# Luoyadan/CRB-active-3Ddet

Hardware: AMD Instinct MI355X
Metric: frames/s SECOND fwd+bwd, KITTI 20k-pt clouds (higher is better)
Workload: dtype f32

## Files before the change

crb-active-3ddet_amd/csrc/rows_gemm4.hip:

```cpp
#include <atomic>
#include <type_traits>
#include <utility>
#include "crb_common.h"
#include "winograd_split.h"
#include "../../include/crb_hip.h"

typedef float f32x4 __attribute__((ext_vector_type(4)));

namespace {

constexpr int NT = 256;

template <typename F, int... I>
__device__ __forceinline__ void static_for_impl(F&& f, std::integer_sequence<int, I...>) {
  (f(std::integral_constant<int, I>{}), ...);
}
template <int N, typename F>
__device__ __forceinline__ void static_for(F&& f) { static_for_impl(f, std::make_integer_sequence<int, N>{}); }

template <int B>
__device__ __forceinline__ void mfma_acc(const bf16x8& A, const bf16x8& Bv) {
  asm volatile("v_mfma_f32_32x32x16_bf16 a[%2:%3], %0, %1, a[%2:%3]" : : "v"(A), "v"(Bv), "n"(B * 16), "n"(B * 16 + 15));
}
template <int R>
__device__ __forceinline__ float acc_read() {
  float x;
  asm volatile("v_accvgpr_read_b32 %0, a[%1]" : "=v"(x) : "n"(R));
  return x;
}
template <int R>
__device__ __forceinline__ void acc_zero() { asm volatile("v_accvgpr_write_b32 a[%0], 0" : : "n"(R)); }
__device__ __forceinline__ void acc_settle() { asm volatile("s_nop 15\n\ts_nop 15" ::: "memory"); }

#define RG_ACC_0_127                                                                                                                   \
  "a0", "a1", "a2", "a3", "a4", "a5", "a6", "a7", "a8", "a9", "a10", "a11", "a12", "a13", "a14", "a15", "a16", "a17", "a18", "a19",   \
      "a20", "a21", "a22", "a23", "a24", "a25", "a26", "a27", "a28", "a29", "a30", "a31", "a32", "a33", "a34", "a35", "a36", "a37",   \
      "a38", "a39", "a40", "a41", "a42", "a43", "a44", "a45", "a46", "a47", "a48", "a49", "a50", "a51", "a52", "a53", "a54", "a55",   \
      "a56", "a57", "a58", "a59", "a60", "a61", "a62", "a63", "a64", "a65", "a66", "a67", "a68", "a69", "a70", "a71", "a72", "a73",   \
      "a74", "a75", "a76", "a77", "a78", "a79", "a80", "a81", "a82", "a83", "a84", "a85", "a86", "a87", "a88", "a89", "a90", "a91",   \
      "a92", "a93", "a94", "a95", "a96", "a97", "a98", "a99", "a100", "a101", "a102", "a103", "a104", "a105", "a106", "a107", "a108", \
      "a109", "a110", "a111", "a112", "a113", "a114", "a115", "a116", "a117", "a118", "a119", "a120", "a121", "a122", "a123", "a124", \
      "a125", "a126", "a127"
#define RG_ACC_128_255                                                                                                                 \
  "a128", "a129", "a130", "a131", "a132", "a133", "a134", "a135", "a136", "a137", "a138", "a139", "a140", "a141", "a142", "a143",     \
      "a144", "a145", "a146", "a147", "a148", "a149", "a150", "a151", "a152", "a153", "a154", "a155", "a156", "a157", "a158", "a159", \
      "a160", "a161", "a162", "a163", "a164", "a165", "a166", "a167", "a168", "a169", "a170", "a171", "a172", "a173", "a174", "a175", \
      "a176", "a177", "a178", "a179", "a180", "a181", "a182", "a183", "a184", "a185", "a186", "a187", "a188", "a189", "a190", "a191", \
      "a192", "a193", "a194", "a195", "a196", "a197", "a198", "a199", "a200", "a201", "a202", "a203", "a204", "a205", "a206", "a207", \
      "a208", "a209", "a210", "a211", "a212", "a213", "a214", "a215", "a216", "a217", "a218", "a219", "a220", "a221", "a222", "a223", \
      "a224", "a225", "a226", "a227", "a228", "a229", "a230", "a231", "a232", "a233", "a234", "a235", "a236", "a237", "a238", "a239", \
      "a240", "a241", "a242", "a243", "a244", "a245", "a246", "a247", "a248", "a249", "a250", "a251", "a252", "a253", "a254", "a255"

__device__ constexpr int pass_a(int p) { return p == 0 ? 0 : p == 1 ? 2 : p == 2 ? 1 : p == 3 ? 0 : p == 4 ? 1 : 0; }
__device__ constexpr int pass_b(int p) { return p == 0 ? 2 : p == 1 ? 0 : p == 2 ? 1 : p == 3 ? 1 : 0; }

struct Split8 {
  float sv[2], s1[2], s2[2];
  u32x4 q0, q1, q2;
  template <int E>
  __device__ __forceinline__ void put(float v) {
    constexpr int hh = E & 1;
    sv[hh] = v;
    split3f(v, s1[hh], s2[hh]);
    if constexpr (hh == 1) {
      q0[E >> 1] = __builtin_amdgcn_perm(__float_as_uint(sv[1]), __float_as_uint(sv[0]), 0x07060302u);
      q1[E >> 1] = __builtin_amdgcn_perm(__float_as_uint(s1[1]), __float_as_uint(s1[0]), 0x07060302u);
      q2[E >> 1] = __builtin_amdgcn_perm(__float_as_uint(s2[1]), __float_as_uint(s2[0]), 0x07060302u);
    }
  }
  __device__ __forceinline__ void get(bf16x8 (&f)[3]) const {
    f[0] = __builtin_bit_cast(bf16x8, q0);
    f[1] = __builtin_bit_cast(bf16x8, q1);
    f[2] = __builtin_bit_cast(bf16x8, q2);
  }
};

__global__ __launch_bounds__(256) void rows_gemm4_weights_kernel(const float* __restrict__ w, int64_t s_ci, int64_t s_co, int64_t s_a,
                                                                 int64_t s_b, unsigned char* __restrict__ img, int cin, int cout, int s,
                                                                 int direction, int K, int N) {
  const int KS = K >> 4;
  const int64_t id = (int64_t)blockIdx.x * 256 + threadIdx.x;
  if (id >= (int64_t)(N >> 5) * KS * 64) return;
  const int lane = (int)(id & 63), r = lane & 31, h = lane >> 5;
  const int ks = (int)((id >> 6) % KS), nb = (int)((id >> 6) / KS);
  const int n = nb * 32 + r, k0 = (ks >> 1) * 32 + h * 16 + (ks & 1) * 8;
  u32x4 q[3];
  unsigned lo[3] = {0, 0, 0};
#pragma unroll
  for (int j = 0; j < 8; ++j) {
    const int k = k0 + j;
    const int ci = direction ? n : k, tc = direction ? k : n;
    const int t = tc / cout, co = tc - t * cout;
    const float v = w[ci * s_ci + co * s_co + (t / s) * s_a + (t % s) * s_b];
    unsigned p[3];
    split3(v, p[0], p[1], p[2]);
#pragma unroll
    for (int i = 0; i < 3; ++i) {
      if (j & 1) q[i][j >> 1] = lo[i] | (p[i] << 16);
      else lo[i] = p[i];
    }
  }
  unsigned char* dst = img + ((int64_t)(nb * KS + ks) * 3) * 1024 + lane * 16;
#pragma unroll
  for (int i = 0; i < 3; ++i) *reinterpret_cast<u32x4*>(dst + i * 1024) = q[i];
}

constexpr int RG_LDS_BYTES = 4 * 32 * 64 * 16;

struct RgArgs {
  const float* x;
  float* y;
  const unsigned char* wimg;
  int M;
  int W, s;
  int kseg, nseg;
  int tin, tout;
  int K, N;
  int ldx, ldy;
  int wrn;
  int col_tiles, tiles;
};

__device__ __forceinline__ unsigned big_pix(int m, int W, int s) { return (unsigned)(s * (m + (s - 1) * W * (m / W))); }

__global__ __launch_bounds__(NT, 1) void rows_gemm4_kernel(RgArgs a) {
  extern __shared__ __attribute__((aligned(16))) unsigned char rg_lds[];
  asm volatile("" ::: RG_ACC_0_127, RG_ACC_128_255);
  const int lane = threadIdx.x & 63, wave = __builtin_amdgcn_readfirstlane(threadIdx.x >> 6);
// ... 410 lines not shown
```

crb-active-3ddet_amd/pcdet/models/backbones_2d/base_bev_backbone.py:

```python
import numpy as np
import torch
import torch.nn as nn

from crbhip import bnrelu

from ...utils.fold_utils import fold_conv_bn
from ...utils.linear_rows import LinearRows, rows_view, rows_to_nchw


ROWS_TRAIN = True
ROWS_GEMM = True
WINOGRAD = __import__('os').environ.get('CRB_WINOGRAD', '1') != '0'


def _wino_fold(w, shift):
    from crbhip import winograd
    return winograd.weights_forward2(w), shift.contiguous()


def _wino_ok(conv, x, pad=None):
    if not WINOGRAD or not isinstance(conv, nn.Conv2d) or not x.is_cuda or x.dtype != torch.float32:
        return False
    from crbhip import winograd
    p = tuple(conv.padding) if pad is None else tuple(pad)
# ... 14 lines not shown
        layer_nums = list(model_cfg.get('LAYER_NUMS', None) or [])
        layer_strides = list(model_cfg.get('LAYER_STRIDES', None) or [])
        num_filters = list(model_cfg.get('NUM_FILTERS', None) or [])
        assert len(layer_nums) == len(layer_strides) == len(num_filters)
        upsample_strides = list(model_cfg.get('UPSAMPLE_STRIDES', None) or [])
        num_upsample_filters = list(model_cfg.get('NUM_UPSAMPLE_FILTERS', None) or [])
        assert len(upsample_strides) == len(num_upsample_filters)
        c_in_list = [input_channels] + num_filters[:-1]
        self.blocks = nn.ModuleList()
        self.deblocks = nn.ModuleList()
        for idx, (c_in, c_out, n, s) in enumerate(zip(c_in_list, num_filters, layer_nums, layer_strides)):
            layers = [nn.ZeroPad2d(1), nn.Conv2d(c_in, c_out, kernel_size=3, stride=s, padding=0, bias=False),
                      _bn(c_out), nn.ReLU()]
            for _ in range(n):
                layers += [nn.Conv2d(c_out, c_out, kernel_size=3, padding=1, bias=False), _bn(c_out), nn.ReLU()]
            self.blocks.append(nn.Sequential(*layers))
            if upsample_strides:
                us, uc = upsample_strides[idx], num_upsample_filters[idx]
                if us >= 1:
                    up = nn.ConvTranspose2d(c_out, uc, us, stride=us, bias=False)
                else:
                    ds = int(np.round(1 / us))
                    up = nn.Conv2d(c_out, uc, ds, stride=ds, bias=False)
                self.deblocks.append(nn.Sequential(up, _bn(uc), nn.ReLU()))
        c_in = sum(num_upsample_filters)
        if len(upsample_strides) > len(layer_nums):
            self.deblocks.append(nn.Sequential(
                nn.ConvTranspose2d(c_in, c_in, upsample_strides[-1], stride=upsample_strides[-1], bias=False),
                _bn(c_in), nn.ReLU()))
        self.num_bev_features = c_in

    @staticmethod
    def _run_folded(seq, x):
        mods = list(seq)
        i = 0
        while i < len(mods):
            m = mods[i]
            pad = None
            if isinstance(m, nn.ZeroPad2d) and i + 1 < len(mods) and isinstance(mods[i + 1], nn.Conv2d):
                c, pd = mods[i + 1], m.padding
                if c.padding == (0, 0) and c.padding_mode == 'zeros' and pd[0] == pd[1] and pd[2] == pd[3]:
                    pad, i, m = (pd[2], pd[0]), i + 1, c
            if isinstance(m, (nn.Conv2d, nn.ConvTranspose2d)) and i + 1 < len(mods) and isinstance(mods[i + 1], nn.BatchNorm2d):
                bn = mods[i + 1]
                relu = i + 2 < len(mods) and isinstance(mods[i + 2], nn.ReLU)
                if _wino_ok(m, x, pad):
                    from crbhip import winograd
                    U, shift = fold_conv_bn(m, bn, _wino_fold)
                    x = winograd.conv3x3_U2(x, U, shift, relu)
                    i += 3 if relu else 2
                    continue
                rows_ok = x.is_cuda and x.is_contiguous(memory_format=torch.channels_last) and m.bias is None
                if rows_ok:
                    y = m(x) if pad is None else torch.nn.functional.conv2d(x, m.weight, None, m.stride, pad, m.dilation,
                                                                             m.groups)
                    rows_ok = y.is_contiguous(memory_format=torch.channels_last) and \
                        bnrelu.supported(y.new_empty((2, y.shape[1])), bn)
                if rows_ok:
                    n, c, h, w_ = y.shape
                    rows = y.permute(0, 2, 3, 1).reshape(n * h * w_, c)
                    z = bnrelu.bn_apply_(rows, bn, relu)
                    x = z.view(n, h, w_, c).permute(0, 3, 1, 2)
                else:
                    w, shift = fold_conv_bn(m, bn)
                    if isinstance(m, nn.Conv2d):
                        x = torch.nn.functional.conv2d(x, w, shift, m.stride, m.padding if pad is None else pad, m.dilation,
                                                       m.groups)
                    else:
                        x = torch.nn.functional.conv_transpose2d(x, w, shift, m.stride, m.padding, m.output_padding,
                                                                 m.groups, m.dilation)
                    if relu:
                        x = torch.relu_(x)
                i += 3 if relu else 2
            else:
                x = m(x) if pad is None else torch.nn.functional.conv2d(x, m.weight, m.bias, m.stride, pad, m.dilation, m.groups)
                i += 1
        return x

    @staticmethod
    def _pad_conv(mods, i, x):
        m = mods[i]
        if isinstance(m, nn.ZeroPad2d) and i + 1 < len(mods) and isinstance(mods[i + 1], nn.Conv2d):
            c = mods[i + 1]
            pd = m.padding
            if c.padding == (0, 0) and c.padding_mode == 'zeros' and pd[0] == pd[1] and pd[2] == pd[3]:
                if _wino_ok(c, x, (pd[2], pd[0])):
                    from crbhip import winograd
                    return BaseBEVBackbone._wino_conv(c, x, mods[i + 2] if i + 2 < len(mods) else None), 2
                if torch.are_deterministic_algorithms_enabled() and torch.is_grad_enabled() and pd[0] == pd[2] and x.is_cuda:
                    from crbhip import dense_strided
                    if dense_strided.supported(c, x):
                        return dense_strided.conv_det(c, x, (pd[2], pd[0])), 2
                return torch.nn.functional.conv2d(x, c.weight, c.bias, c.stride, (pd[2], pd[0]), c.dilation, c.groups), 2
        return None, 0

    @staticmethod
    def _wino_conv(conv, x, nxt):
        from crbhip import winograd
        if winograd.STATS and conv.bias is None and isinstance(nxt, nn.BatchNorm2d) and nxt.training and \
                nxt.momentum is not None and bnrelu.FUSE_RUNNING and torch.is_grad_enabled() and not bnrelu.frame_groups_active():
            y, slabs = winograd.conv3x3_stats(x, conv.weight)
            y._crb_bn_slabs = slabs
            return y
        return winograd.conv3x3(x, conv.weight, conv.bias)

    @staticmethod
    def _run_rows_train(seq, x):
        mods = list(seq)
        i = 0
        while i < len(mods):
            m = mods[i]
            nxt = mods[i + 1] if i + 1 < len(mods) else None
            y, used = BaseBEVBackbone._pad_conv(mods, i, x)
            if used:
                x, i = y, i + used
                continue
            if _wino_ok(m, x):
                x = BaseBEVBackbone._wino_conv(m, x, nxt)
                i += 1
                continue
            if isinstance(m, nn.BatchNorm2d) and isinstance(nxt, nn.ReLU) and \
                    x.is_contiguous(memory_format=torch.channels_last) and \
                    bnrelu.supported(x.new_empty((2, x.shape[1])), m):
                n, c, h, w_ = x.shape
                rows = x.permute(0, 2, 3, 1).reshape(n * h * w_, c)
                slabs = getattr(x, '_crb_bn_slabs', None)
                x = bnrelu.bn_relu(rows, m, relu=True, slabs=slabs).view(n, h, w_, c).permute(0, 3, 1, 2)
                i += 2
            else:
                x = m(x)
                i += 1
        return x

    @staticmethod
    def _up(conv, x):
        if ROWS_GEMM and x.is_cuda:
            from crbhip import rows_gemm
            y = rows_gemm.up_conv(conv, x)
            if y is not None:
                return y
        if ROWS_GEMM and x.is_cuda and conv.bias is None and conv.kernel_size == (1, 1) and conv.stride == (1, 1) and \
# ... 98 lines not shown
```

include/crb_hip.h:

```cpp
#ifndef CRB_HIP_H
#define CRB_HIP_H
#include <stdint.h>

#ifdef __cplusplus
extern "C" {
#endif

#define CRB_OK 0
#define CRB_ERR_ARG (-1)
#define CRB_ERR_WORKSPACE (-2)
#define CRB_ERR_LAUNCH (-3)
#define CRB_ERR_UNSUPPORTED (-4)

int crb_abi_version(void);

int64_t crb_voxelize_workspace_bytes(int64_t n_points, int B, int max_voxels, int max_points);
int crb_voxelize(const float* points, int64_t n_points, int num_features,
                 const int32_t* frame_offsets, int B,
                 const float* range_min_xyz, const float* voxel_size_xyz, const int32_t* grid_xyz,
                 int max_voxels, int max_points,
                 float* voxels, int32_t* coords, int32_t* num_points, float* mean_features,
                 int32_t* num_voxels_out,
                 void* workspace, int64_t workspace_bytes, void* stream);

// ... 385 lines not shown
int64_t crb_winograd2_stats_slabs(int N, int H, int W);
int crb_conv3x3_winograd2_stats_nhwc(const float* x, const float* U, float* y, float* stats, int N, int H, int W, int cin, int cout,
                                     void* stream);

int crb_winograd4_supported(int cin, int cout, int H, int W);
int64_t crb_winograd4_weights_bytes(int cin, int cout);
int crb_winograd4_weights_conv(const float* w, int64_t so, int64_t si, int64_t sky, int64_t skx, void* U, int conv_cin, int conv_cout,
                               int mode, void* stream);
int crb_winograd4_weights_conv_multi(int n, const float* const* w, const int64_t* strides, void* const* U, const int32_t* conv_cin,
                                     const int32_t* conv_cout, const int32_t* mode, void* stream);
int crb_conv3x3_winograd4_nhwc(const float* x, const void* U, float* y, int N, int H, int W, int cin, int cout, const float* bias,
                               int relu, void* stream);
int64_t crb_winograd4_stats_slabs(int N, int H, int W);
int crb_conv3x3_winograd4_stats_nhwc(const float* x, const void* U, float* y, float* stats, int N, int H, int W, int cin, int cout,
                                     void* stream);
int crb_winograd4c_supported(int cin, int cout, int H, int W);
int crb_conv3x3_winograd4c_nhwc(const float* x, const void* U, float* y, int N, int H, int W, int cin, int cout,
                                const float* bias, int relu, void* stream);
int64_t crb_winograd4c_stats_slabs(int N, int H, int W);
int crb_conv3x3_winograd4c_stats_nhwc(const float* x, const void* U, float* y, float* stats, int N, int H, int W, int cin,
                                      int cout, void* stream);

int crb_bev_blocks_geometry(int N, int H, int W, int32_t* geom);
int64_t crb_bev_blocks_ints(int N, int H, int W);
int crb_bev_blocks(const int32_t* indices, int64_t n, int N, int H, int W, int32_t* out, int64_t out_ints, void* stream);
int crb_conv3x3_winograd4c_blocks_nhwc(const float* x, const void* U, float* y, float* stats, int N, int H, int W, int cin,
                                       int cout, const int32_t* list, const int32_t* count, const int32_t* rest,
                                       const int32_t* rest_count, void* stream);

int crb_winograd2_wgrad_supported(int cin, int cout, int H, int W);
int64_t crb_winograd2_wgrad_workspace_bytes(int cin, int cout);
int crb_winograd2_wgrad(const float* x, const float* dy, float* dw, int64_t so, int64_t si, int64_t sky, int64_t skx,
                        int N, int H, int W, int cin, int cout, void* workspace, int64_t workspace_bytes, void* stream);
int crb_winograd4_wgrad_supported(int cin, int cout, int H, int W);
int64_t crb_winograd4_wgrad_workspace_bytes(int cin, int cout);
int crb_winograd4_wgrad(const float* x, const float* dy, float* dw, int64_t so, int64_t si, int64_t sky, int64_t skx,
                        int N, int H, int W, int cin, int cout, void* workspace, int64_t workspace_bytes, void* stream);
int crb_winograd4_wgrad_blocks(const float* x, const float* dy, float* dw, int64_t so, int64_t si, int64_t sky, int64_t skx,
                               int N, int H, int W, int cin, int cout, const int32_t* list, const int32_t* count,
                               void* workspace, int64_t workspace_bytes, void* stream);

int crb_rows_gemm4_supported(int cin, int cout, int stride, int direction);
int64_t crb_rows_gemm4_weights_bytes(int cin, int cout, int stride);
int crb_rows_gemm4_weights(const float* w, int64_t s_ci, int64_t s_co, int64_t s_a, int64_t s_b, void* image, int cin, int cout,
                           int stride, int direction, void* stream);
int crb_rows_gemm4_forward(const float* x, const void* image, float* y, int N, int H, int W, int cin, int cout, int stride,
                           void* stream);
int crb_rows_gemm4_input_grad(const float* dy, const void* image, float* dx, int N, int H, int W, int cin, int cout, int stride,
                              void* stream);
int64_t crb_rows_gemm4_wgrad_workspace_bytes(int cin, int cout, int stride);
int crb_rows_gemm4_wgrad(const float* x, const float* dy, float* dw, int64_t s_ci, int64_t s_co, int64_t s_a, int64_t s_b, int N,
                         int H, int W, int cin, int cout, int stride, void* workspace, int64_t workspace_bytes, void* stream);

int crb_cu_reservation(int cus, void* stream);

int crb_bev_interpolate_forward(const float* bev, int B, int H, int W, int C, const float* keypoints, int64_t M, float x_min,
                                float y_min, float voxel_x, float voxel_y, float bev_stride, float* out, void* stream);
int crb_bev_interpolate_backward(const float* dout, int B, int H, int W, int C, const float* keypoints, int64_t M, float x_min,
                                 float y_min, float voxel_x, float voxel_y, float bev_stride, float* dbev, void* stream);

int crb_roi_bev_pool(const float* bev, int B, int H, int W, int C, const float* rois, int roi_row_stride, int R, int grid_size,
                     double x_min, double y_min, double cell_x, double cell_y, float* out, void* stream);

int crb_voxel_pool_supported(int C, int nsample);
int crb_voxel_query(const float* xyz, int64_t N, const float* new_xyz, const int32_t* new_coords, int64_t M, int B,
                    const int32_t* shape_dhw, const int32_t* ranges_zyx, float radius, int nsample, const int64_t* hkeys,
                    const int32_t* hvals, int64_t capacity, int32_t* idx, int32_t* cnt, void* stream);
int64_t crb_voxel_pool_moments_workspace_bytes(int64_t M);
int crb_voxel_pool_moments(const float* xyz, const float* new_xyz, const int32_t* idx, const int32_t* cnt, int64_t M, int nsample,
                           double* sums, void* workspace, int64_t workspace_bytes, void* stream);
int crb_voxel_pool_forward(const float* features_in, int64_t N, int C, const float* xyz, const float* new_xyz, const int32_t* idx,
                           const int32_t* cnt, int64_t M, int nsample, int pool, const float* A, const float* b, float* out,
                           void* stream);
int64_t crb_voxel_pool_backward_workspace_bytes(int64_t M, int C);
int crb_voxel_pool_backward(const float* grad_out, const float* features_in, int64_t N, int C, const float* xyz,
                            const float* new_xyz, const int32_t* idx, const int32_t* cnt, int64_t M, int nsample, int pool,
                            const float* A, const float* b, float* d_features, float* g_sel, int32_t* a_row, float* d_Ab,
                            void* workspace, int64_t workspace_bytes, void* stream);

int crb_pillar_vfe_supported(int C, int T, int Cout);
int crb_pillar_vfe_num_moments(int C);
int64_t crb_pillar_vfe_moments_workspace_bytes(int64_t M, int C);
int crb_pillar_vfe_moments(const float* voxels, const int32_t* num_points, const int32_t* coords, int64_t M, int T, int C,
                           const float* voxel_size, const float* offsets, double* sums, void* workspace, int64_t workspace_bytes,
                           void* stream);
int crb_pillar_vfe_forward(const float* voxels, const int32_t* num_points, const int32_t* coords, int64_t M, int T, int C,
                           const float* voxel_size, const float* offsets, const float* A, const float* b, int Cout, float* out,
                           void* stream);
int64_t crb_pillar_vfe_backward_workspace_bytes(int64_t M, int C, int Cout);
int crb_pillar_vfe_backward(const float* grad_out, const float* voxels, const int32_t* num_points, const int32_t* coords, int64_t M,
                            int T, int C, const float* voxel_size, const float* offsets, const float* A, const float* b, int Cout,
                            double* d_sums, void* workspace, int64_t workspace_bytes, void* stream);

#define CRB_LOSSNET_MAX_LAYERS 4
typedef struct CrbLossNetArgs {
  const float* x[CRB_LOSSNET_MAX_LAYERS];
  const float* w[CRB_LOSSNET_MAX_LAYERS];
  const float* gamma[CRB_LOSSNET_MAX_LAYERS];
  const float* beta[CRB_LOSSNET_MAX_LAYERS];
  float* running_mean[CRB_LOSSNET_MAX_LAYERS];
  float* running_var[CRB_LOSSNET_MAX_LAYERS];
  int64_t* num_batches_tracked[CRB_LOSSNET_MAX_LAYERS];
  int32_t channels[CRB_LOSSNET_MAX_LAYERS];
  int32_t num_layer;
  int32_t rows_per_frame;
  int32_t frames;
// ... 110 lines not shown
```

Baseline: 492.7.

## Add MFMA implicit-GEMM kernel for stride-2 3x3 convs in BEV backbone

Adds a custom HIP kernel for the bias-free 3x3 stride-2 padding-1 downsampling convolutions in the BEV backbone. It uses an implicit GEMM on bf16 MFMA with a three-way split of the f32 values, and handles the input gradient by decomposing it into four output-parity classes, each with its own tap subset. Weight images are cached per tensor version. By default only the input-gradient direction is switched on; forward and weight gradient still use the vendor convolution. Shared MFMA helpers move into a common header. The aim is to replace vendor strided-conv backward with a tuned kernel, at the cost of extra weight-image preparation and a more complex code path.

```diff
diff --git a/crb-active-3ddet_amd/crbhip/conv_s2.py b/crb-active-3ddet_amd/crbhip/conv_s2.py
--- /dev/null
+++ b/crb-active-3ddet_amd/crbhip/conv_s2.py
@@ -0,0 +1,204 @@
+import os
+
+import numpy as np
+import torch
+
+from ._lib import lib, check, ptr, cur_stream, require_cuda, CrbHipError
+
+KERNEL = os.environ.get('CRB_CONV_S2_KERNEL', 'x6')
+DEFAULT_LAUNCHES = 'i'
+LAUNCHES = set(v.strip() for v in os.environ.get('CRB_CONV_S2_LAUNCHES', DEFAULT_LAUNCHES).split(',') if v.strip())
+FORWARD, INPUT_GRAD, WGRAD = 0, 1, 2
+_DIR = 'fiw'
+TAPS_FORWARD = tuple((ky, kx) for ky in range(3) for kx in range(3))
+CLASSES = ((1, 1), (1, 0), (0, 1), (0, 0))
+
+
+def class_taps(ph, pw):
+    return tuple((ky, kx) for ky in ((0, 2) if ph else (1,)) for kx in ((0, 2) if pw else (1,)))
+
+
+TAPS_INPUT_GRAD = tuple(t for ph, pw in CLASSES for t in class_taps(ph, pw))
+
+
+def supported(cin, cout, direction):
+    return bool(lib.crb_conv_s2_supported(int(cin), int(cout), int(direction)))
+
+
+def use(cin, cout, direction):
+    return KERNEL == 'x6' and _DIR[direction] in LAUNCHES and supported(cin, cout, direction)
+
+
+def _geometry(conv, pad=None):
+    import torch.nn as nn
+    if not isinstance(conv, nn.Conv2d) or conv.bias is not None or conv.groups != 1 or conv.dilation != (1, 1):
+        return None
+    p = tuple(conv.padding) if pad is None else tuple(pad)
+    if conv.kernel_size != (3, 3) or conv.stride != (2, 2) or p != (1, 1) or conv.padding_mode != 'zeros':
+        return None
+    if pad is not None and tuple(conv.padding) != (0, 0):
+        return None
+    return conv.in_channels, conv.out_channels
+
+
+def dispatch(conv, x, pad=None):
+    g = _geometry(conv, pad)
+    if KERNEL != 'x6':
+        return 'vendor', 'CRB_CONV_S2_KERNEL=%s' % KERNEL
+    if g is None:
+        return 'vendor', 'not a bias-free 3x3 stride 2 padding 1 convolution'
+    if not (x.is_cuda and x.dim() == 4 and x.dtype == torch.float32 and x.is_contiguous(memory_format=torch.channels_last)):
+        return 'vendor', 'input is not an f32 channels_last device map'
+    cin, cout = g
+    if x.shape[1] != cin or x.shape[0] * x.shape[2] * x.shape[3] * max(cin, cout) >= 2 ** 31:
+        return 'vendor', 'map of %s does not fit the kernels\' 32-bit element index' % (tuple(x.shape),)
+    on = [d for d in range(3) if use(cin, cout, d)]
+    if not on:
+        return 'vendor', 'no direction of %d -> %d is switched on with an instance' % (cin, cout)
+    return 'x6', ''.join(_DIR[d] for d in on)
+
+
+_IMAGES = {}
+
+
+def weights(weight, cin, cout, direction):
+    require_cuda(weight)
+    w = weight.detach()
+    key = (w.data_ptr(), w.device.index, int(direction))
+    tag = (w._version, tuple(w.shape), tuple(w.stride()), cin, cout)
+    hit = _IMAGES.get(key)
+    if hit is not None and hit[0] == tag:
+        return hit[1]
+    if w.dtype != torch.float32 or tuple(w.shape) != (cout, cin, 3, 3):
+        raise CrbHipError('crb_conv_s2_weights takes an f32 (Cout, Cin, 3, 3) weight')
+    img = torch.empty((int(lib.crb_conv_s2_weights_bytes(cin, cout)),), dtype=torch.uint8, device=w.device)
+    s_co, s_ci, s_ky, s_kx = w.stride()
+    check(lib.crb_conv_s2_weights(w.data_ptr(), s_co, s_ci, s_ky, s_kx, ptr(img), cin, cout, int(direction), cur_stream(w.device)),
+          'crb_conv_s2_weights')
+    if len(_IMAGES) > 64:
+        _IMAGES.clear()
+    _IMAGES[key] = (tag, img, w)
+    return img
+
+
+def weight_matrix_reference(w, direction):
+    w = np.asarray(w)
+    if direction == FORWARD:
+        return np.concatenate([w[:, :, ky, kx].T for ky, kx in TAPS_FORWARD], axis=0)
+    return np.concatenate([w[:, :, ky, kx] for ky, kx in TAPS_INPUT_GRAD], axis=0)
+
+
+def weight_image_reference(w, direction):
+    wm = np.ascontiguousarray(weight_matrix_reference(np.asarray(w, dtype=np.float32), direction))
+    K, N = wm.shape
+    ks, lane, j = np.meshgrid(np.arange(K // 16), np.arange(64), np.arange(8), indexing='ij')
+    k = 32 * (ks >> 1) + 16 * (lane >> 5) + 8 * (ks & 1) + j
+    r = lane & 31
+    out = np.empty((N // 32, K // 16, 3, 64, 8), dtype=np.uint16)
+    for nb in range(N // 32):
+        v = np.ascontiguousarray(wm[k, 32 * nb + r])
+        for p in range(3):
+            hi = v.view(np.uint32) & np.uint32(0xffff0000)
+            out[nb, :, p] = (hi >> np.uint32(16)).astype(np.uint16)
+            v = v - hi.view(np.float32)
+    return out
+
+
+def forward_rows(N, H, W):
+    Ho, Wo = (H + 1) // 2, (W + 1) // 2
+    n, ho, wo = np.meshgrid(np.arange(N), np.arange(Ho), np.arange(Wo), indexing='ij')
+    src, valid = [], []
+    for ky, kx in TAPS_FORWARD:
+        h, w = 2 * ho - 1 + ky, 2 * wo - 1 + kx
+        valid.append(((h >= 0) & (h < H) & (w >= 0) & (w < W)).reshape(-1))
+        src.append(((n * H + np.clip(h, 0, H - 1)) * W + np.clip(w, 0, W - 1)).reshape(-1))
+    return np.stack(src), np.stack(valid)
+
+
+def input_grad_rows(N, H, W, ph, pw):
+    Ho, Wo = (H + 1) // 2, (W + 1) // 2
+    Hr, Wr = (H + 1 - ph) // 2, (W + 1 - pw) // 2
+    n, hr, wr = np.meshgrid(np.arange(N), np.arange(Hr), np.arange(Wr), indexing='ij')
+    dst = ((n * H + 2 * hr + ph) * W + 2 * wr + pw).reshape(-1)
+    src, valid = [], []
+    for ky, kx in class_taps(ph, pw):
+        ho, wo = hr + (1 if ky == 0 else 0), wr + (1 if kx == 0 else 0)
+        valid.append(((ho < Ho) & (wo < Wo)).reshape(-1))
+        src.append(((n * Ho + np.minimum(ho, Ho - 1)) * Wo + np.minimum(wo, Wo - 1)).reshape(-1))
+    return dst, np.stack(src), np.stack(valid)
+
+
+def _nhwc(x):
+    if not x.is_contiguous(memory_format=torch.channels_last):
+        x = x.contiguous(memory_format=torch.channels_last)
+    return x.permute(0, 2, 3, 1)
+
+
+def forward_x6(x, weight, cin, cout):
+    require_cuda(x, weight)
+    xv = _nhwc(x)
+    N, H, W, _ = xv.shape
+    img = weights(weight, cin, cout, FORWARD)
+    y = torch.empty((N, cout, (H + 1) // 2, (W + 1) // 2), dtype=torch.float32, device=x.device, memory_format=torch.channels_last)
+    check(lib.crb_conv_s2_forward(xv.data_ptr(), ptr(img), y.data_ptr(), N, H, W, cin, cout, cur_stream(x.device)), 'crb_conv_s2_forward')
+    return y
+
+
+def input_grad_x6(dy, weight, cin, cout, H, W):
+    require_cuda(dy, weight)
+    gv = _nhwc(dy)
+    N = gv.shape[0]
+    if tuple(gv.shape) != (N, (H + 1) // 2, (W + 1) // 2, cout):
+        raise CrbHipError('conv_s2 input gradient: dy does not belong to a %d x %d map' % (H, W))
+    img = weights(weight, cin, cout, INPUT_GRAD)
+    dx = torch.empty((N, cin, H, W), dtype=torch.float32, device=dy.device, memory_format=torch.channels_last)
+    check(lib.crb_conv_s2_input_grad(gv.data_ptr(), ptr(img), dx.data_ptr(), N, H, W, cin, cout, cur_stream(dy.device)),
+          'crb_conv_s2_input_grad')
+    return dx
+
+
+class _ConvS2(torch.autograd.Function):
+
+    @staticmethod
+    def forward(ctx, x, weight, cin, cout, det_wgrad=False):
+        ctx.save_for_backward(x, weight)
+        ctx.geo = (cin, cout)
+        ctx.det_wgrad = det_wgrad
+        if use(cin, cout, FORWARD):
+            return forward_x6(x, weight, cin, cout)
+        return torch.nn.functional.conv2d(x, weight, None, 2, 1)
+
+    @staticmethod
+    def backward(ctx, dy):
+        x, weight = ctx.saved_tensors
+        cin, cout = ctx.geo
+        dy = dy.contiguous(memory_format=torch.channels_last)
+        dx = dw = None
+        if ctx.needs_input_grad[0]:
+            if use(cin, cout, INPUT_GRAD):
+                dx = input_grad_x6(dy, weight, cin, cout, x.shape[2], x.shape[3])
+            else:
+                dx = torch.ops.aten.convolution_backward(dy, x, weight, None, [2, 2], [1, 1], [1, 1], False, [0, 0], 1,
+                                                         [True, False, False])[0]
+        if ctx.needs_input_grad[1]:
+            if ctx.det_wgrad:
+                from . import dense_strided
+                dw = dense_strided.weight_grad('conv', x, dy, 3, 3, 2, 1)
+            else:
+                dw = torch.ops.aten.convolution_backward(dy, x, weight, None, [2, 2], [1, 1], [1, 1], False, [0, 0], 1,
+                                                         [False, True, False])[1]
+        return dx, dw, None, None, None
+
+
+def conv(conv_module, x, pad=None):
+    path, _ = dispatch(conv_module, x, pad)
+    if path != 'x6':
+        return None
+    cin, cout = _geometry(conv_module, pad)
+    det_wgrad = False
+    if torch.are_deterministic_algorithms_enabled() and torch.is_grad_enabled():
+        from . import dense_strided
+        if not (use(cin, cout, FORWARD) and use(cin, cout, INPUT_GRAD) and dense_strided.supported(conv_module, x)):
+            return None
+        det_wgrad = True
+    return _ConvS2.apply(x, conv_module.weight, cin, cout, det_wgrad)
diff --git a/crb-active-3ddet_amd/csrc/conv_s2_rows.hip b/crb-active-3ddet_amd/csrc/conv_s2_rows.hip
--- /dev/null
+++ b/crb-active-3ddet_amd/csrc/conv_s2_rows.hip
@@ -0,0 +1,353 @@
+#include <atomic>
+#include <climits>
+#include "rows_gemm_common.h"
+#include "../../include/crb_hip.h"
+
+namespace {
+
+constexpr int CS_FLUSH = 8;
+constexpr int CS_LDS_BYTES = 4 * 32 * 64 * 16;
+constexpr int CS_SEGS = 4;
+
+__host__ constexpr int cs_geo(int nth, int ntw, int dh0, int sh, int dw0, int sw, int ph, int pw) {
+  return ntw | nth << 2 | (dh0 + 1) << 4 | (sh + 1) << 6 | (dw0 + 1) << 8 | (sw + 1) << 10 | ph << 12 | pw << 13;
+}
+
+struct CsArgs {
+  const float* x;
+  float* y;
+  const unsigned char* wimg;
+  int Hs, Ws, Hd, Wd;
+  int as, bs;
+  int kch, nch;
+  int wrn, col_tiles, tiles;
+  int tile0[CS_SEGS];
+  int M[CS_SEGS];
+  int Hr[CS_SEGS], Wr[CS_SEGS];
+  int geo[CS_SEGS];
+  int tap0[CS_SEGS];
+};
+
+struct CsSeg {
+  int tile0, M, Hr, Wr, ntw, dh0, sh, dw0, sw, ph, pw, KC, ks0;
+};
+
+__device__ __forceinline__ CsSeg cs_seg(const CsArgs& a, int tile) {
+  const int si = (tile >= a.tile0[1]) + (tile >= a.tile0[2]) + (tile >= a.tile0[3]);
+  auto pick = [&](const int (&v)[CS_SEGS]) __attribute__((always_inline)) { return si == 0 ? v[0] : si == 1 ? v[1] : si == 2 ? v[2] : v[3]; };
+  CsSeg s;
+  const int g = pick(a.geo);
+  s.tile0 = pick(a.tile0); s.M = pick(a.M); s.Hr = pick(a.Hr); s.Wr = pick(a.Wr); s.ks0 = pick(a.tap0) * (a.kch >> 4);
+  s.ntw = g & 3;
+  s.dh0 = ((g >> 4) & 3) - 1; s.sh = ((g >> 6) & 3) - 1;
+  s.dw0 = ((g >> 8) & 3) - 1; s.sw = ((g >> 10) & 3) - 1;
+  s.ph = (g >> 12) & 1; s.pw = (g >> 13) & 1;
+  s.KC = ((g >> 2) & 3) * s.ntw * (a.kch >> 5);
+  return s;
+}
+
+__global__ __launch_bounds__(NT, 1) void conv_s2_rows_kernel(CsArgs a) {
+  extern __shared__ __attribute__((aligned(16))) unsigned char cs_lds[];
+  asm volatile("" ::: RG_ACC_0_127, RG_ACC_128_255);
+  const int lane = threadIdx.x & 63, wave = __builtin_amdgcn_readfirstlane(threadIdx.x >> 6);
+  const int wr = wave % a.wrn, wc = wave / a.wrn, r = lane & 31, h = lane >> 5;
+  const int tile_rows = a.wrn * 64, tile_cols = (4 / a.wrn) * 128;
+  const int kcs = a.kch >> 5, KS = 18 * kcs;
+  int lt = blockIdx.x, lc = 0;
+  if (lt >= a.tiles) return;
+  const unsigned char* const wl = a.wimg + lane * 16;
+  CsSeg cur = cs_seg(a, lt);
+
+  static_for<256>([](auto rc) { acc_zero<decltype(rc)::value>(); });
+
+  int rn[2], rh[2], rw[2];
+  auto set_rows = [&](int tile, const CsSeg& s) __attribute__((always_inline)) {
+#pragma unroll
+    for (int rb = 0; rb < 2; ++rb) {
+      const int m = min(((tile - s.tile0) / a.col_tiles) * tile_rows + wr * 64 + rb * 32 + r, s.M - 1);
+      const int n = m / (s.Hr * s.Wr), rem = m - n * (s.Hr * s.Wr), hr = rem / s.Wr;
+      rn[rb] = n * a.Hs;
+      rh[rb] = a.as * hr;
+      rw[rb] = a.as * (rem - hr * s.Wr);
+    }
+  };
+  auto load_a = [&](int c, const CsSeg& s, f32x4 (&dst)[2][4], bool (&ok)[2]) __attribute__((always_inline)) {
+    const int t = c / kcs, cs = c - t * kcs, th = t / s.ntw, tw = t - th * s.ntw;
+    const int dh = s.dh0 + s.sh * th, dw = s.dw0 + s.sw * tw;
+#pragma unroll
+    for (int rb = 0; rb < 2; ++rb) {
+      const int hs = rh[rb] + dh, ws = rw[rb] + dw;
+      ok[rb] = (unsigned)hs < (unsigned)a.Hs && (unsigned)ws < (unsigned)a.Ws;
+      const int hc = min(max(hs, 0), a.Hs - 1), wcl = min(max(ws, 0), a.Ws - 1);
+      const float* p = a.x + ((size_t)(rn[rb] + hc) * a.Ws + wcl) * a.kch + cs * 32 + h * 16;
+#pragma unroll
+      for (int q = 0; q < 4; ++q) dst[rb][q] = *reinterpret_cast<const f32x4*>(p + 4 * q);
+    }
+  };
+  auto load_b = [&](int tile, const CsSeg& s, int ks, bf16x8 (&dst)[4][3]) __attribute__((always_inline)) {
+    const int nb0 = (((tile - s.tile0) % a.col_tiles) * tile_cols + wc * 128) >> 5;
+#pragma unroll
+    for (int cb = 0; cb < 4; ++cb)
+#pragma unroll
+      for (int p = 0; p < 3; ++p)
+        dst[cb][p] = *reinterpret_cast<const bf16x8*>(wl + ((size_t)((nb0 + cb) * KS + s.ks0 + ks) * 3 + p) * 1024);
+  };
+  auto step = [&](const bf16x8 (&Bw)[4][3], const bf16x8 (&Xf)[2][3], auto&& gap) __attribute__((always_inline)) {
+    static_for<48>([&](auto kc) __attribute__((always_inline)) {
+      constexpr int k = decltype(kc)::value, cb = k / 12, rb = (k / 6) & 1, pass = k % 6;
+      mfma_acc<(pass == 5 ? 0 : 8) + 4 * rb + cb>(Bw[cb][pass_a(pass)], Xf[rb][pass_b(pass)]);
+      gap(kc);
+      __builtin_amdgcn_sched_barrier(0);
+    });
+  };
+
+  f32x4 Ahi[2][2];
+  bool okhi[2];
+  bf16x8 XF0[2][3], B0[4][3];
+  set_rows(lt, cur);
+  {
+    f32x4 A0[2][4];
+    load_a(0, cur, A0, okhi);
+    load_b(lt, cur, 0, B0);
+#pragma unroll
+    for (int rb = 0; rb < 2; ++rb) {
+      Split8 sp;
+      static_for<8>([&](auto ec) { constexpr int e = decltype(ec)::value; sp.put<e>(okhi[rb] ? A0[rb][e >> 2][e & 3] : 0.f); });
+      sp.get(XF0[rb]);
+      Ahi[rb][0] = A0[rb][2];
+      Ahi[rb][1] = A0[rb][3];
+    }
+  }
+  asm volatile("s_nop 4" ::: "memory");
+
+  for (;;) {
+    int nt = lt, nc = lc + 1;
+    if (nc == cur.KC) { nc = 0; nt = lt + (int)gridDim.x; }
+    const bool more = nt < a.tiles;
+    if (!more) { nt = lt; nc = lc; }
+    CsSeg nxt = cur;
+    if (nt != lt) nxt = cs_seg(a, nt);
+    bf16x8 B1[4][3];
+    load_b(lt, cur, 2 * lc + 1, B1);
+    if (nt != lt) set_rows(nt, nxt);
+    f32x4 An[2][4];
+    bool okn[2];
+    load_a(nc, nxt, An, okn);
+    __builtin_amdgcn_sched_barrier(0);
+
+    bf16x8 XF1[2][3];
+    Split8 sp;
+    step(B0, XF0, [&](auto kc) __attribute__((always_inline)) {
+      constexpr int k = decltype(kc)::value;
+      if constexpr (k < 16) {
+        constexpr int rb = k >> 3, e = k & 7;
+        sp.put<e>(okhi[rb] ? Ahi[rb][e >> 2][e & 3] : 0.f);
+        if constexpr (e == 7) sp.get(XF1[rb]);
+      }
+    });
+    load_b(nt, nxt, 2 * nc, B0);
+    __builtin_amdgcn_sched_barrier(0);
+    step(B1, XF1, [&](auto kc) __attribute__((always_inline)) {
+      constexpr int k = decltype(kc)::value;
+      if constexpr (k >= 24 && k < 40) {
+        constexpr int rb = (k - 24) >> 3, e = (k - 24) & 7;
+        sp.put<e>(okn[rb] ? An[rb][e >> 2][e & 3] : 0.f);
+        if constexpr (e == 7) sp.get(XF0[rb]);
+      }
+    });
+
+    if (lc != cur.KC - 1 && (lc + 1) % CS_FLUSH == 0) {
+      f32x4* const part = reinterpret_cast<f32x4*>(cs_lds) + wave * (32 * 64) + lane;
+      const bool first = lc + 1 == CS_FLUSH;
+      acc_settle();
+      static_for<32>([&](auto qc) __attribute__((always_inline)) {
+        constexpr int R0 = 4 * decltype(qc)::value;
+        f32x4 v = (f32x4){acc_read<R0>(), acc_read<R0 + 1>(), acc_read<R0 + 2>(), acc_read<R0 + 3>()};
+        if (!first) v += part[decltype(qc)::value * 64];
+        part[decltype(qc)::value * 64] = v;
+      });
+      static_for<128>([](auto rc) { acc_zero<decltype(rc)::value>(); });
+      asm volatile("s_nop 4" ::: "memory");
+    }
+    if (lc == cur.KC - 1) {
+      const int tl = lt - cur.tile0;
+      const int col0 = (tl % a.col_tiles) * tile_cols + wc * 128;
+      const bool parts = cur.KC > CS_FLUSH;
+      acc_settle();
+      static_for<2>([&](auto rbc) __attribute__((always_inline)) {
+        constexpr int rb = decltype(rbc)::value;
+        const int m = (tl / a.col_tiles) * tile_rows + wr * 64 + rb * 32 + r;
+        const bool ok = m < cur.M;
+        const int mm = min(m, cur.M - 1);
+        const int n = mm / (cur.Hr * cur.Wr), rem = mm - n * (cur.Hr * cur.Wr), hr = rem / cur.Wr, wq = rem - hr * cur.Wr;
+        const int pix = (n * a.Hd + a.bs * hr + cur.ph) * a.Wd + a.bs * wq + cur.pw;
+        float* const out = a.y + (size_t)pix * a.nch + col0 + 4 * h;
+        static_for<16>([&](auto qc) __attribute__((always_inline)) {
+          constexpr int cb = decltype(qc)::value >> 2, j = decltype(qc)::value & 3, R0 = (4 * rb + cb) * 16 + 4 * j;
+          f32x4 v = (f32x4){acc_read<R0>() + acc_read<128 + R0>(), acc_read<R0 + 1>() + acc_read<129 + R0>(),
+                            acc_read<R0 + 2>() + acc_read<130 + R0>(), acc_read<R0 + 3>() + acc_read<131 + R0>()};
+          if (parts) v += (reinterpret_cast<const f32x4*>(cs_lds) + wave * (32 * 64) + lane)[(R0 / 4) * 64];
+          if (ok) *reinterpret_cast<f32x4*>(out + cb * 32 + 8 * j) = v;
+        });
+      });
+      static_for<256>([](auto rc) { acc_zero<decltype(rc)::value>(); });
+      asm volatile("s_nop 4" ::: "memory");
+    }
+    if (!more) break;
+#pragma unroll
+    for (int rb = 0; rb < 2; ++rb) {
+      Ahi[rb][0] = An[rb][2];
+      Ahi[rb][1] = An[rb][3];
+      okhi[rb] = okn[rb];
+    }
+    lt = nt;
+    lc = nc;
+    cur = nxt;
+  }
+}
+
+constexpr unsigned long long CS_ORDER_FWD = 0x876543210ULL;
+constexpr unsigned long long CS_ORDER_IGRAD = 0x453718620ULL;
+
+__global__ __launch_bounds__(256) void conv_s2_weights_kernel(const float* __restrict__ w, int64_t s_k, int64_t s_n, int64_t s_ky,
+                                                              int64_t s_kx, unsigned char* __restrict__ img, int kch, int nch,
+                                                              unsigned long long order) {
+  const int KS = (9 * kch) >> 4;
+  const int64_t id = (int64_t)blockIdx.x * 256 + threadIdx.x;
+  if (id >= (int64_t)(nch >> 5) * KS * 64) return;
+  const int lane = (int)(id & 63), r = lane & 31, h = lane >> 5;
+  const int ks = (int)((id >> 6) % KS), nb = (int)((id >> 6) / KS);
+  const int n = nb * 32 + r, k0 = (ks >> 1) * 32 + h * 16 + (ks & 1) * 8;
+  u32x4 q[3];
+  unsigned lo[3] = {0, 0, 0};
+#pragma unroll
+  for (int j = 0; j < 8; ++j) {
+    const int k = k0 + j;
+    const int t = k / kch, kc = k - t * kch, tap = (int)((order >> (4 * t)) & 15), ky = tap / 3, kx = tap - 3 * ky;
+    const float v = w[kc * s_k + n * s_n + ky * s_ky + kx * s_kx];
+    unsigned p[3];
+    split3(v, p[0], p[1], p[2]);
+#pragma unroll
+    for (int i = 0; i < 3; ++i) {
+      if (j & 1) q[i][j >> 1] = lo[i] | (p[i] << 16);
+      else lo[i] = p[i];
+    }
+  }
+  unsigned char* dst = img + ((int64_t)(nb * KS + ks) * 3) * 1024 + lane * 16;
+#pragma unroll
+  for (int i = 0; i < 3; ++i) *reinterpret_cast<u32x4*>(dst + i * 1024) = q[i];
+}
+
+__host__ int cs_cu_count() {
+  static std::atomic<int> n_cu{0};
+  int n = n_cu.load(std::memory_order_relaxed);
+  if (!n) {
+    int dev = 0;
+    hipDeviceProp_t prop;
+    if (hipGetDevice(&dev) != hipSuccess || hipGetDeviceProperties(&prop, dev) != hipSuccess) return 256;
+    n = prop.multiProcessorCount > 0 ? prop.multiProcessorCount : 256;
+    n_cu.store(n, std::memory_order_relaxed);
+  }
+  return n;
+}
+
+__host__ bool cs_sizes_ok(int N, int H, int W, int cin, int cout) {
+  if (N <= 0 || H <= 0 || W <= 0) return false;
+  return (int64_t)N * H * W * (cin > cout ? cin : cout) < (1LL << 31);
+}
+
+constexpr int CS_PH[CS_SEGS] = {1, 1, 0, 0}, CS_PW[CS_SEGS] = {1, 0, 1, 0};
+
+__host__ int cs_launch(CsArgs& a, int nsegs, void* stream) {
+  a.wrn = a.nch % 256 == 0 ? 2 : 4;
+  const int tile_rows = a.wrn * 64, tile_cols = (4 / a.wrn) * 128;
+  a.col_tiles = a.nch / tile_cols;
+  int64_t tiles = 0;
+  for (int s = 0; s < CS_SEGS; ++s) {
+    if (s >= nsegs) { a.tile0[s] = INT_MAX; a.M[s] = 0; a.Hr[s] = a.Wr[s] = 1; a.geo[s] = a.geo[0]; a.tap0[s] = 0; continue; }
+    a.tile0[s] = (int)tiles;
+    tiles += (((int64_t)a.M[s] + tile_rows - 1) / tile_rows) * a.col_tiles;
+    if (tiles >= (1LL << 30)) return CRB_ERR_ARG;
+  }
+  a.tiles = (int)tiles;
+  if (!a.tiles) return CRB_OK;
+  const int grid = a.tiles < cs_cu_count() ? a.tiles : cs_cu_count();
+  static std::atomic<unsigned> attr_done[64];
+  int dev = 0;
+  CRB_HIP(hipGetDevice(&dev));
+  if (dev < 0 || dev >= 64) return CRB_ERR_ARG;
+  if (!attr_done[dev].load(std::memory_order_acquire)) {
+    CRB_HIP(hipFuncSetAttribute((const void*)conv_s2_rows_kernel, hipFuncAttributeMaxDynamicSharedMemorySize, CS_LDS_BYTES));
+    attr_done[dev].store(1u, std::memory_order_release);
+  }
+  hipLaunchKernelGGL(conv_s2_rows_kernel, dim3((unsigned)grid), dim3(NT), CS_LDS_BYTES, (hipStream_t)stream, a);
+  CRB_CHECK_LAUNCH();
+  return CRB_OK;
+}
+
+}
+
+extern "C" int crb_conv_s2_supported(int cin, int cout, int direction) {
+  const bool n_ok = cout == 128 || cout == 256;
+  if (direction == 0) return ((cin == 64 || cin == 128) && n_ok) ? 1 : 0;
+  if (direction == 1) return (cin == 128 && n_ok) ? 1 : 0;
+  return 0;
+}
+
+extern "C" int64_t crb_conv_s2_weights_bytes(int cin, int cout) {
+  if (!crb_conv_s2_supported(cin, cout, 0) && !crb_conv_s2_supported(cin, cout, 1)) return 0;
+  return (int64_t)9 * cin * cout * 6;
+}
+
+extern "C" int crb_conv_s2_weights(const float* w, int64_t s_co, int64_t s_ci, int64_t s_ky, int64_t s_kx, void* image, int cin, int cout,
+                                   int direction, void* stream) {
+  if (direction != 0 && direction != 1) return CRB_ERR_ARG;
+  if (!crb_conv_s2_supported(cin, cout, direction)) return CRB_ERR_UNSUPPORTED;
+  if (!w || !image) return CRB_ERR_ARG;
+  const int kch = direction ? cout : cin, nch = direction ? cin : cout;
+  const int64_t threads = (int64_t)(nch / 32) * (9 * kch / 16) * 64;
+  hipLaunchKernelGGL(conv_s2_weights_kernel, dim3((unsigned)((threads + 255) / 256)), dim3(256), 0, (hipStream_t)stream, w,
+                     direction ? s_co : s_ci, direction ? s_ci : s_co, s_ky, s_kx, (unsigned char*)image, kch, nch,
+                     direction ? CS_ORDER_IGRAD : CS_ORDER_FWD);
+  CRB_CHECK_LAUNCH();
+  return CRB_OK;
+}
+
+extern "C" int crb_conv_s2_forward(const float* x, const void* image, float* y, int N, int H, int W, int cin, int cout, void* stream) {
+  if (N <= 0 || H <= 0 || W <= 0 || !x || !image || !y) return CRB_ERR_ARG;
+  if (!crb_conv_s2_supported(cin, cout, 0)) return CRB_ERR_UNSUPPORTED;
+  if (!cs_sizes_ok(N, H, W, cin, cout)) return CRB_ERR_ARG;
+  const int Ho = (H + 1) / 2, Wo = (W + 1) / 2;
+  CsArgs a;
+  a.x = x; a.y = y; a.wimg = (const unsigned char*)image;
+  a.Hs = H; a.Ws = W; a.Hd = Ho; a.Wd = Wo;
+  a.as = 2; a.bs = 1;
+  a.kch = cin; a.nch = cout;
+  a.M[0] = N * Ho * Wo; a.Hr[0] = Ho; a.Wr[0] = Wo;
+  a.geo[0] = cs_geo(3, 3, -1, 1, -1, 1, 0, 0);
+  a.tap0[0] = 0;
+  return cs_launch(a, 1, stream);
+}
+
+extern "C" int crb_conv_s2_input_grad(const float* dy, const void* image, float* dx, int N, int H, int W, int cin, int cout,
+                                      void* stream) {
+  if (N <= 0 || H <= 0 || W <= 0 || !dy || !image || !dx) return CRB_ERR_ARG;
+  if (!crb_conv_s2_supported(cin, cout, 1)) return CRB_ERR_UNSUPPORTED;
+  if (!cs_sizes_ok(N, H, W, cin, cout)) return CRB_ERR_ARG;
+  const int Ho = (H + 1) / 2, Wo = (W + 1) / 2;
+  CsArgs a;
+  a.x = dy; a.y = dx; a.wimg = (const unsigned char*)image;
+  a.Hs = Ho; a.Ws = Wo; a.Hd = H; a.Wd = W;
+  a.as = 1; a.bs = 2;
+  a.kch = cout; a.nch = cin;
+  int tap0 = 0;
+  for (int s = 0; s < CS_SEGS; ++s) {
+    const int ph = CS_PH[s], pw = CS_PW[s];
+    const int Hr = (H + 1 - ph) / 2, Wr = (W + 1 - pw) / 2;
+    a.M[s] = N * Hr * Wr; a.Hr[s] = Hr > 0 ? Hr : 1; a.Wr[s] = Wr > 0 ? Wr : 1;
+    a.geo[s] = cs_geo(1 + ph, 1 + pw, ph, -1, pw, -1, ph, pw);
+    a.tap0[s] = tap0;
+    tap0 += (1 + ph) * (1 + pw);
+  }
+  return cs_launch(a, CS_SEGS, stream);
+}
diff --git a/crb-active-3ddet_amd/csrc/rows_gemm4.hip b/crb-active-3ddet_amd/csrc/rows_gemm4.hip
--- a/crb-active-3ddet_amd/csrc/rows_gemm4.hip
+++ b/crb-active-3ddet_amd/csrc/rows_gemm4.hip
@@ -5,75 +5,9 @@
 #include "winograd_split.h"
 #include "../../include/crb_hip.h"
 
-typedef float f32x4 __attribute__((ext_vector_type(4)));
+#include "rows_gemm_common.h"
 
 namespace {
-
-constexpr int NT = 256;
-
-template <typename F, int... I>
-__device__ __forceinline__ void static_for_impl(F&& f, std::integer_sequence<int, I...>) {
-  (f(std::integral_constant<int, I>{}), ...);
-}
-template <int N, typename F>
-__device__ __forceinline__ void static_for(F&& f) { static_for_impl(f, std::make_integer_sequence<int, N>{}); }
-
-template <int B>
-__device__ __forceinline__ void mfma_acc(const bf16x8& A, const bf16x8& Bv) {
-  asm volatile("v_mfma_f32_32x32x16_bf16 a[%2:%3], %0, %1, a[%2:%3]" : : "v"(A), "v"(Bv), "n"(B * 16), "n"(B * 16 + 15));
-}
-template <int R>
-__device__ __forceinline__ float acc_read() {
-  float x;
-  asm volatile("v_accvgpr_read_b32 %0, a[%1]" : "=v"(x) : "n"(R));
-  return x;
-}
-template <int R>
-__device__ __forceinline__ void acc_zero() { asm volatile("v_accvgpr_write_b32 a[%0], 0" : : "n"(R)); }
-__device__ __forceinline__ void acc_settle() { asm volatile("s_nop 15\n\ts_nop 15" ::: "memory"); }
-
-#define RG_ACC_0_127                                                                                                                   \
-  "a0", "a1", "a2", "a3", "a4", "a5", "a6", "a7", "a8", "a9", "a10", "a11", "a12", "a13", "a14", "a15", "a16", "a17", "a18", "a19",   \
-      "a20", "a21", "a22", "a23", "a24", "a25", "a26", "a27", "a28", "a29", "a30", "a31", "a32", "a33", "a34", "a35", "a36", "a37",   \
-      "a38", "a39", "a40", "a41", "a42", "a43", "a44", "a45", "a46", "a47", "a48", "a49", "a50", "a51", "a52", "a53", "a54", "a55",   \
-      "a56", "a57", "a58", "a59", "a60", "a61", "a62", "a63", "a64", "a65", "a66", "a67", "a68", "a69", "a70", "a71", "a72", "a73",   \
-      "a74", "a75", "a76", "a77", "a78", "a79", "a80", "a81", "a82", "a83", "a84", "a85", "a86", "a87", "a88", "a89", "a90", "a91",   \
-      "a92", "a93", "a94", "a95", "a96", "a97", "a98", "a99", "a100", "a101", "a102", "a103", "a104", "a105", "a106", "a107", "a108", \
-      "a109", "a110", "a111", "a112", "a113", "a114", "a115", "a116", "a117", "a118", "a119", "a120", "a121", "a122", "a123", "a124", \
-      "a125", "a126", "a127"
-#define RG_ACC_128_255                                                                                                                 \
-  "a128", "a129", "a130", "a131", "a132", "a133", "a134", "a135", "a136", "a137", "a138", "a139", "a140", "a141", "a142", "a143",     \
-      "a144", "a145", "a146", "a147", "a148", "a149", "a150", "a151", "a152", "a153", "a154", "a155", "a156", "a157", "a158", "a159", \
-      "a160", "a161", "a162", "a163", "a164", "a165", "a166", "a167", "a168", "a169", "a170", "a171", "a172", "a173", "a174", "a175", \
-      "a176", "a177", "a178", "a179", "a180", "a181", "a182", "a183", "a184", "a185", "a186", "a187", "a188", "a189", "a190", "a191", \
-      "a192", "a193", "a194", "a195", "a196", "a197", "a198", "a199", "a200", "a201", "a202", "a203", "a204", "a205", "a206", "a207", \
-      "a208", "a209", "a210", "a211", "a212", "a213", "a214", "a215", "a216", "a217", "a218", "a219", "a220", "a221", "a222", "a223", \
-      "a224", "a225", "a226", "a227", "a228", "a229", "a230", "a231", "a232", "a233", "a234", "a235", "a236", "a237", "a238", "a239", \
-      "a240", "a241", "a242", "a243", "a244", "a245", "a246", "a247", "a248", "a249", "a250", "a251", "a252", "a253", "a254", "a255"
-
-__device__ constexpr int pass_a(int p) { return p == 0 ? 0 : p == 1 ? 2 : p == 2 ? 1 : p == 3 ? 0 : p == 4 ? 1 : 0; }
-__device__ constexpr int pass_b(int p) { return p == 0 ? 2 : p == 1 ? 0 : p == 2 ? 1 : p == 3 ? 1 : 0; }
-
-struct Split8 {
-  float sv[2], s1[2], s2[2];
-  u32x4 q0, q1, q2;
-  template <int E>
-  __device__ __forceinline__ void put(float v) {
-    constexpr int hh = E & 1;
-    sv[hh] = v;
-    split3f(v, s1[hh], s2[hh]);
-    if constexpr (hh == 1) {
-      q0[E >> 1] = __builtin_amdgcn_perm(__float_as_uint(sv[1]), __float_as_uint(sv[0]), 0x07060302u);
-      q1[E >> 1] = __builtin_amdgcn_perm(__float_as_uint(s1[1]), __float_as_uint(s1[0]), 0x07060302u);
-      q2[E >> 1] = __builtin_amdgcn_perm(__float_as_uint(s2[1]), __float_as_uint(s2[0]), 0x07060302u);
-    }
-  }
-  __device__ __forceinline__ void get(bf16x8 (&f)[3]) const {
-    f[0] = __builtin_bit_cast(bf16x8, q0);
-    f[1] = __builtin_bit_cast(bf16x8, q1);
-    f[2] = __builtin_bit_cast(bf16x8, q2);
-  }
-};
 
 __global__ __launch_bounds__(256) void rows_gemm4_weights_kernel(const float* __restrict__ w, int64_t s_ci, int64_t s_co, int64_t s_a,
                                                                  int64_t s_b, unsigned char* __restrict__ img, int cin, int cout, int s,
diff --git a/crb-active-3ddet_amd/csrc/rows_gemm_common.h b/crb-active-3ddet_amd/csrc/rows_gemm_common.h
--- /dev/null
+++ b/crb-active-3ddet_amd/csrc/rows_gemm_common.h
@@ -0,0 +1,77 @@
+#pragma once
+#include <type_traits>
+#include <utility>
+#include "crb_common.h"
+#include "winograd_split.h"
+
+typedef float f32x4 __attribute__((ext_vector_type(4)));
+
+namespace {
+
+constexpr int NT = 256;
+
+template <typename F, int... I>
+__device__ __forceinline__ void static_for_impl(F&& f, std::integer_sequence<int, I...>) {
+  (f(std::integral_constant<int, I>{}), ...);
+}
+template <int N, typename F>
+__device__ __forceinline__ void static_for(F&& f) { static_for_impl(f, std::make_integer_sequence<int, N>{}); }
+
+template <int B>
+__device__ __forceinline__ void mfma_acc(const bf16x8& A, const bf16x8& Bv) {
+  asm volatile("v_mfma_f32_32x32x16_bf16 a[%2:%3], %0, %1, a[%2:%3]" : : "v"(A), "v"(Bv), "n"(B * 16), "n"(B * 16 + 15));
+}
+template <int R>
+__device__ __forceinline__ float acc_read() {
+  float x;
+  asm volatile("v_accvgpr_read_b32 %0, a[%1]" : "=v"(x) : "n"(R));
+  return x;
+}
+template <int R>
+__device__ __forceinline__ void acc_zero() { asm volatile("v_accvgpr_write_b32 a[%0], 0" : : "n"(R)); }
+__device__ __forceinline__ void acc_settle() { asm volatile("s_nop 15\n\ts_nop 15" ::: "memory"); }
+
+#define RG_ACC_0_127                                                                                                                   \
+  "a0", "a1", "a2", "a3", "a4", "a5", "a6", "a7", "a8", "a9", "a10", "a11", "a12", "a13", "a14", "a15", "a16", "a17", "a18", "a19",   \
+      "a20", "a21", "a22", "a23", "a24", "a25", "a26", "a27", "a28", "a29", "a30", "a31", "a32", "a33", "a34", "a35", "a36", "a37",   \
+      "a38", "a39", "a40", "a41", "a42", "a43", "a44", "a45", "a46", "a47", "a48", "a49", "a50", "a51", "a52", "a53", "a54", "a55",   \
+      "a56", "a57", "a58", "a59", "a60", "a61", "a62", "a63", "a64", "a65", "a66", "a67", "a68", "a69", "a70", "a71", "a72", "a73",   \
+      "a74", "a75", "a76", "a77", "a78", "a79", "a80", "a81", "a82", "a83", "a84", "a85", "a86", "a87", "a88", "a89", "a90", "a91",   \
+      "a92", "a93", "a94", "a95", "a96", "a97", "a98", "a99", "a100", "a101", "a102", "a103", "a104", "a105", "a106", "a107", "a108", \
+      "a109", "a110", "a111", "a112", "a113", "a114", "a115", "a116", "a117", "a118", "a119", "a120", "a121", "a122", "a123", "a124", \
+      "a125", "a126", "a127"
+#define RG_ACC_128_255                                                                                                                 \
+  "a128", "a129", "a130", "a131", "a132", "a133", "a134", "a135", "a136", "a137", "a138", "a139", "a140", "a141", "a142", "a143",     \
+      "a144", "a145", "a146", "a147", "a148", "a149", "a150", "a151", "a152", "a153", "a154", "a155", "a156", "a157", "a158", "a159", \
+      "a160", "a161", "a162", "a163", "a164", "a165", "a166", "a167", "a168", "a169", "a170", "a171", "a172", "a173", "a174", "a175", \
+      "a176", "a177", "a178", "a179", "a180", "a181", "a182", "a183", "a184", "a185", "a186", "a187", "a188", "a189", "a190", "a191", \
+      "a192", "a193", "a194", "a195", "a196", "a197", "a198", "a199", "a200", "a201", "a202", "a203", "a204", "a205", "a206", "a207", \
+      "a208", "a209", "a210", "a211", "a212", "a213", "a214", "a215", "a216", "a217", "a218", "a219", "a220", "a221", "a222", "a223", \
+      "a224", "a225", "a226", "a227", "a228", "a229", "a230", "a231", "a232", "a233", "a234", "a235", "a236", "a237", "a238", "a239", \
+      "a240", "a241", "a242", "a243", "a244", "a245", "a246", "a247", "a248", "a249", "a250", "a251", "a252", "a253", "a254", "a255"
+
+__device__ constexpr int pass_a(int p) { return p == 0 ? 0 : p == 1 ? 2 : p == 2 ? 1 : p == 3 ? 0 : p == 4 ? 1 : 0; }
+__device__ constexpr int pass_b(int p) { return p == 0 ? 2 : p == 1 ? 0 : p == 2 ? 1 : p == 3 ? 1 : 0; }
+
+struct Split8 {
+  float sv[2], s1[2], s2[2];
+  u32x4 q0, q1, q2;
+  template <int E>
+  __device__ __forceinline__ void put(float v) {
+    constexpr int hh = E & 1;
+    sv[hh] = v;
+    split3f(v, s1[hh], s2[hh]);
+    if constexpr (hh == 1) {
+      q0[E >> 1] = __builtin_amdgcn_perm(__float_as_uint(sv[1]), __float_as_uint(sv[0]), 0x07060302u);
+      q1[E >> 1] = __builtin_amdgcn_perm(__float_as_uint(s1[1]), __float_as_uint(s1[0]), 0x07060302u);
+      q2[E >> 1] = __builtin_amdgcn_perm(__float_as_uint(s2[1]), __float_as_uint(s2[0]), 0x07060302u);
+    }
+  }
+  __device__ __forceinline__ void get(bf16x8 (&f)[3]) const {
+    f[0] = __builtin_bit_cast(bf16x8, q0);
+    f[1] = __builtin_bit_cast(bf16x8, q1);
+    f[2] = __builtin_bit_cast(bf16x8, q2);
+  }
+};
+
+}
diff --git a/crb-active-3ddet_amd/pcdet/models/backbones_2d/base_bev_backbone.py b/crb-active-3ddet_amd/pcdet/models/backbones_2d/base_bev_backbone.py
--- a/crb-active-3ddet_amd/pcdet/models/backbones_2d/base_bev_backbone.py
+++ b/crb-active-3ddet_amd/pcdet/models/backbones_2d/base_bev_backbone.py
@@ -90,8 +90,10 @@
                     continue
                 rows_ok = x.is_cuda and x.is_contiguous(memory_format=torch.channels_last) and m.bias is None
                 if rows_ok:
-                    y = m(x) if pad is None else torch.nn.functional.conv2d(x, m.weight, None, m.stride, pad, m.dilation,
-                                                                             m.groups)
+                    y = BaseBEVBackbone._conv_s2(m, x, pad)
+                    if y is None:
+                        y = m(x) if pad is None else torch.nn.functional.conv2d(x, m.weight, None, m.stride, pad, m.dilation,
+                                                                                 m.groups)
                     rows_ok = y.is_contiguous(memory_format=torch.channels_last) and \
                         bnrelu.supported(y.new_empty((2, y.shape[1])), bn)
                 if rows_ok:
@@ -116,6 +118,13 @@
         return x
 
     @staticmethod
+    def _conv_s2(conv, x, pad):
+        if not x.is_cuda or not isinstance(conv, nn.Conv2d) or conv.stride != (2, 2):
+            return None
+        from crbhip import conv_s2
+        return conv_s2.conv(conv, x, pad)
+
+    @staticmethod
     def _pad_conv(mods, i, x):
         m = mods[i]
         if isinstance(m, nn.ZeroPad2d) and i + 1 < len(mods) and isinstance(mods[i + 1], nn.Conv2d):
@@ -125,6 +134,9 @@
                 if _wino_ok(c, x, (pd[2], pd[0])):
                     from crbhip import winograd
                     return BaseBEVBackbone._wino_conv(c, x, mods[i + 2] if i + 2 < len(mods) else None), 2
+                y = BaseBEVBackbone._conv_s2(c, x, (pd[2], pd[0]))
+                if y is not None:
+                    return y, 2
                 if torch.are_deterministic_algorithms_enabled() and torch.is_grad_enabled() and pd[0] == pd[2] and x.is_cuda:
                     from crbhip import dense_strided
                     if dense_strided.supported(c, x):
diff --git a/include/crb_hip.h b/include/crb_hip.h
--- a/include/crb_hip.h
+++ b/include/crb_hip.h
@@ -461,6 +461,13 @@
 int crb_rows_gemm4_wgrad(const float* x, const float* dy, float* dw, int64_t s_ci, int64_t s_co, int64_t s_a, int64_t s_b, int N,
                          int H, int W, int cin, int cout, int stride, void* workspace, int64_t workspace_bytes, void* stream);
 
+int crb_conv_s2_supported(int cin, int cout, int direction);
+int64_t crb_conv_s2_weights_bytes(int cin, int cout);
+int crb_conv_s2_weights(const float* w, int64_t s_co, int64_t s_ci, int64_t s_ky, int64_t s_kx, void* image, int cin, int cout,
+                        int direction, void* stream);
+int crb_conv_s2_forward(const float* x, const void* image, float* y, int N, int H, int W, int cin, int cout, void* stream);
+int crb_conv_s2_input_grad(const float* dy, const void* image, float* dx, int N, int H, int W, int cin, int cout, void* stream);
+
 int crb_cu_reservation(int cus, void* stream);
 
 int crb_bev_interpolate_forward(const float* bev, int B, int H, int W, int C, const float* keypoints, int64_t M, float x_min,
```

Result: no change. 497.0 (median of 6 runs) (+0.9%).
